# TimoLassmann/tagdust

Hardware: AMD Instinct MI355X
Metric: reads/s (150 bp, 8-barcode arch) (higher is better)
Workload: dtype f32

## Files before the change

tagdust_amd/csrc/td_api.hip:

```cpp
#include <math.h>
#include <stdarg.h>
#include <stdlib.h>
#include <string.h>
#include <unistd.h>

#include <mutex>
#include <thread>

#include "../../include/tagdust_model.h"
#include "td_ctx.h"
#include "td_model_flat.h"
#include "td_stats.h"

static std::string g_create_error;

static int g_hwq_user = 0;
static bool g_hwq_late = false;
static bool kfd_is_open()
{
	char path[64], target[64];
	for (int fd = 0; fd < 256; fd++) {
		snprintf(path, sizeof path, "/proc/self/fd/%d", fd);
		const ssize_t n = readlink(path, target, sizeof target - 1);
		if (n <= 0) continue;
// ... 10 lines not shown
}

int fail(td_ctx* c, const char* fmt, ...)
{
	char buf[512];
	va_list ap;
	va_start(ap, fmt);
	vsnprintf(buf, sizeof buf, fmt, ap);
	va_end(ap);
	if (c) c->err = buf; else g_create_error = buf;
	return TD_FAIL;
}

extern "C" const char* td_last_error(const td_ctx* ctx)
{
	return ctx ? ctx->err.c_str() : g_create_error.c_str();
}

extern "C" void td_stream_release(void);
static std::mutex g_live_mu;
static int g_live_ctx = 0;

extern "C" int td_ctx_create(int device, td_ctx** out)
{
	if (!out) return fail(nullptr, "td_ctx_create: out is NULL");
	*out = nullptr;
	int ndev = 0;
	hipError_t e = hipGetDeviceCount(&ndev);
	if (e != hipSuccess || ndev <= 0)
		return fail(nullptr, "td_ctx_create: no HIP device available (%s) -- this library has no CPU path",
		            e == hipSuccess ? "device count 0" : hipGetErrorString(e));
	if (device < 0 || device >= ndev) return fail(nullptr, "td_ctx_create: device %d out of range (0..%d)", device, ndev - 1);
	td_ctx* c = new td_ctx();
	c->device = device;
	hipDeviceProp_t prop;
	if (hipSetDevice(device) != hipSuccess || hipGetDeviceProperties(&prop, device) != hipSuccess) {
		delete c;
		return fail(nullptr, "td_ctx_create: cannot select device %d", device);
	}
	if (strncmp(prop.gcnArchName, "gfx950", 6) != 0) {
		std::string arch = prop.gcnArchName;
		delete c;
		return fail(nullptr, "td_ctx_create: device %d is %s; this library is built for gfx950 (MI355X) only", device, arch.c_str());
	}
	c->n_cu = prop.multiProcessorCount;
	if (const char* e = getenv("TD_SPECIALIZE")) c->spec.specialize = atoi(e) != 0;
	if (const char* e = getenv("TD_OVERLAP")) c->overlap = atoi(e) != 0;
	if (const char* e = getenv("TD_COMPACT_EGRESS")) c->compact_egress = atoi(e) != 0;
	if (const char* e = getenv("TD_RLE_CAP")) { const int v = atoi(e); if (v >= 1 && v <= 127) c->rle_cap_forced = v; }
	if (getenv("TD_NO_LENGTH_CLASSES")) c->length_classes = 0;
	if (getenv("TD_DEBUG_WAIT")) c->debug_wait = 1;
	if (getenv("TD_DEBUG_ALLOC")) c->debug_alloc = 1;
	if (const char* e = getenv("TD_WAVE_SLOTS")) { const long v = atol(e); if (v > 0) c->wave_slots_forced = v; }
	if (const char* e = getenv("TD_WS_CANDIDATES")) c->ws_candidates = atoi(e);
	if (const char* e = getenv("TD_SPEC_LSUM_LIMIT")) c->spec.lsum_limit = atof(e);
	if (getenv("TD_SPEC_SELFCHECK_FAIL")) c->spec.selfcheck_fail = 1;
	if (const char* e = getenv("TD_ASYNC_COMPILE")) c->spec.async_compile = atoi(e) != 0;
	c->hbm_total = prop.totalGlobalMem;
	bool ok = hipStreamCreateWithFlags(&c->stream, hipStreamNonBlocking) == hipSuccess &&
	          hipMalloc((void**)&c->d_logsum, sizeof(float) * TD_LOGSUM_LIVE) == hipSuccess &&
	          hipMalloc((void**)&c->d_counters, sizeof(unsigned long long) * TD_COUNTER_WORDS) == hipSuccess &&
	          hipMemcpy(c->d_logsum, td_logsum_table(), sizeof(float) * TD_LOGSUM_LIVE, hipMemcpyHostToDevice) == hipSuccess &&
	          hipMemset(c->d_counters, 0, sizeof(unsigned long long) * TD_COUNTER_WORDS) == hipSuccess;
	if (!ok) {
		td_ctx_destroy(c);
		return fail(nullptr, "td_ctx_create: HIP resource allocation failed: %s", hipGetErrorString(hipGetLastError()));
	}
	{ std::lock_guard<std::mutex> lk(g_live_mu); g_live_ctx++; c->counted = true; }
	*out = c;
	return TD_OK;
}

void free_dev_model(DevModel& d)
{
	void* p[] = { d.d_hdr, d.d_cols, d.d_hinfo, d.d_pred_off, d.d_pred_idx };
	for (void* q : p) if (q) (void)hipFree(q);
	d = DevModel();
}

extern "C" void td_ctx_destroy(td_ctx* c)
{
	if (!c) return;
	spec_retire_jobs(c, true);
	(void)hipSetDevice(c->device);
	hipStream_t streams[] = { c->stream, c->stream2, c->s_aux, c->s_fin, c->s_up, c->s_down };
	for (hipStream_t st : streams) if (st) (void)hipStreamSynchronize(st);
	free_dev_model(c->dev);
	census_release(c);
	mol_release(c);
	samples_release(c);
	void* bufs[] = { c->d_logsum, c->d_counters, c->d_ws, c->d_art_text, c->d_art_index, c->d_art_pk, c->d_art_seq, c->d_art_hits,
	                 c->spec.d_prune, c->d_tile_next, c->d_ws2, c->d_tile_next2 };
	for (void* p : bufs) if (p) (void)hipFree(p);
	for (int k = 0; k < TD_MAX_PIPELINE; k++) slot_release(c->slots[k]);
	if (c->ev_origin) (void)hipEventDestroy(c->ev_origin);
	(void)spec_unload(c);
	for (hipStream_t st : streams) if (st) (void)hipStreamDestroy(st);
	bool last = false;
	if (c->counted) { std::lock_guard<std::mutex> lk(g_live_mu); last = --g_live_ctx == 0; }
	delete c;
	if (last) td_stream_release();
}

int build_dev_model(td_ctx* c, const td_model_desc* m, DevModel& out)
{
	TdFlatModel f;
	std::string why;
	if (!td_flatten_model(m, f, why)) return fail(c, "%s", why.c_str());
	DevModel d;
	d.h = f.h;
	bool ok = hipMalloc((void**)&d.d_hdr, sizeof f.h) == hipSuccess && hipMalloc((void**)&d.d_cols, sizeof(TdCol) * f.cols.size()) == hipSuccess &&
	          hipMalloc((void**)&d.d_hinfo, sizeof(uint32_t) * f.hinfo.size()) == hipSuccess &&
	          hipMalloc((void**)&d.d_pred_off, sizeof(int32_t) * f.pred_off.size()) == hipSuccess &&
	          hipMalloc((void**)&d.d_pred_idx, sizeof(int32_t) * f.pred_idx.size()) == hipSuccess &&
	          hipMemcpy(d.d_hdr, &f.h, sizeof f.h, hipMemcpyHostToDevice) == hipSuccess &&
	          hipMemcpy(d.d_cols, f.cols.data(), sizeof(TdCol) * f.cols.size(), hipMemcpyHostToDevice) == hipSuccess &&
	          hipMemcpy(d.d_hinfo, f.hinfo.data(), sizeof(uint32_t) * f.hinfo.size(), hipMemcpyHostToDevice) == hipSuccess &&
	          hipMemcpy(d.d_pred_off, f.pred_off.data(), sizeof(int32_t) * f.pred_off.size(), hipMemcpyHostToDevice) == hipSuccess &&
	          hipMemcpy(d.d_pred_idx, f.pred_idx.data(), sizeof(int32_t) * f.pred_idx.size(), hipMemcpyHostToDevice) == hipSuccess;
	if (!ok) { free_dev_model(d); return fail(c, "td_model_upload: device tables: %s", hipGetErrorString(hipGetLastError())); }
	out = d;
	return TD_OK;
}

extern "C" int td_model_upload(td_ctx* c, const td_model_desc* m)
{
	if (!c || !m) return fail(c, "td_model_upload: NULL argument");
	HIPCHK(c, hipSetDevice(c->device));
	if (tickets_outstanding(c)) return fail(c, "td_model_upload: td_submit tickets are outstanding (td_wait them first)");
	spec_retire_jobs(c, false);
	DevModel dm;
	if (build_dev_model(c, m, dm) != TD_OK) return TD_FAIL;
	c->have_model = false;
	for (int k = 0; k < TD_MAX_PIPELINE; k++) { c->slots[k].staged = false; c->slots[k].ran = false; }
	HIPCHK(c, sync_compute(c));
	census_release(c);
	mol_release(c);
	samples_release(c);
	free_dev_model(c->dev);
	c->dev = dm;
	c->model.assign(m);
	c->half_slots = false;
	if (spec_model_uploaded(c) != TD_OK) return TD_FAIL;
	c->have_model = true;
	return TD_OK;
}

extern "C" int td_set_option(td_ctx* c, const char* name, int32_t value)
{
	if (!c || !name) return TD_FAIL;
	if (!strcmp(name, "specialize")) {
		c->spec.specialize = value != 0;
		return TD_OK;
	}
	if (!strcmp(name, "poison_workspace")) { c->poison = value != 0; return TD_OK; }
	if (!strcmp(name, "async_compile")) { c->spec.async_compile = value != 0; return TD_OK; }
	if (!strcmp(name, "spec_probe")) { c->spec.probe = value != 0; return TD_OK; }
	if (!strcmp(name, "compact_egress")) { c->compact_egress = value != 0; return TD_OK; }
	if (!strcmp(name, "stable_input")) {
		if (tickets_outstanding(c)) return fail(c, "td_set_option: stable_input cannot change while tickets are outstanding");
		c->stable_input = value != 0;
		return TD_OK;
	}
	if (!strcmp(name, "length_classes_enabled")) { c->length_classes = value != 0; return TD_OK; }
	if (!strcmp(name, "debug_wait")) { c->debug_wait = value != 0; return TD_OK; }
	if (!strcmp(name, "spec_lsum_limit")) { c->spec.lsum_limit = value > 0 ? (double)value : 1.0e6; return TD_OK; }
	if (!strcmp(name, "rle_cap")) {
		if (value < 0 || value > 127) return fail(c, "td_set_option: rle_cap must be 0 (default) .. 127");
		c->rle_cap_forced = value;
		return TD_OK;
	}
	if (!strcmp(name, "host_threads")) {
		if (value < 1 || value > 16) return fail(c, "td_set_option: host_threads must be 1..16");
		c->host_threads = value;
		return TD_OK;
	}
	if (!strcmp(name, "overlap_decode")) {
		if (tickets_outstanding(c)) return fail(c, "td_set_option: overlap_decode cannot change while tickets are outstanding");
		c->overlap = value != 0; c->submit_parity = 0;
		return TD_OK;
	}
	if (!strcmp(name, "pipeline_depth")) {
		if (value < 1 || value > TD_MAX_PIPELINE) return fail(c, "td_set_option: pipeline_depth must be 1..%d", TD_MAX_PIPELINE);
		if (tickets_outstanding(c)) return fail(c, "td_set_option: pipeline_depth cannot change while tickets are outstanding");
		c->pipeline_depth = value; c->next_slot = 0;
		return TD_OK;
	}
	return fail(c, "td_set_option: unknown option %s", name);
}

extern "C" int td_get_option(td_ctx* c, const char* name, int32_t* value)
{
	if (!c || !name || !value) return TD_FAIL;
	if (!strcmp(name, "specialize")) { *value = c->spec.specialize; return TD_OK; }
	if (!strcmp(name, "spec_lsum_clamped")) { *value = c->spec.ready && !c->spec.oob; return TD_OK; }
	if (!strcmp(name, "pipeline_depth")) { *value = c->pipeline_depth; return TD_OK; }
	if (!strcmp(name, "async_compile")) { *value = c->spec.async_compile; return TD_OK; }
	if (!strcmp(name, "spec_probe")) { *value = c->spec.probe; return TD_OK; }
	if (!strcmp(name, "spec_state")) { *value = spec_state_now(c); return TD_OK; }
	if (!strcmp(name, "spec_batches_generic")) { *value = c->spec.batches_generic; return TD_OK; }
	if (!strcmp(name, "spec_compiles_started")) { *value = td_spec_compiles_started(); return TD_OK; }
	if (!strcmp(name, "spec_probe_us")) { *value = c->spec.probe_us; return TD_OK; }
	if (!strcmp(name, "host_threads")) { *value = c->host_threads; return TD_OK; }
	if (!strcmp(name, "artifacts_active")) { *value = c->art_n > 0; return TD_OK; }
	if (!strcmp(name, "dust")) { *value = c->dust; return TD_OK; }
	if (!strcmp(name, "length_classes")) { *value = c->slots[c->last_slot].n_big; return TD_OK; }
	if (!strcmp(name, "overlap_decode")) { *value = c->overlap; return TD_OK; }
	if (!strcmp(name, "compact_egress")) { *value = c->compact_egress; return TD_OK; }
	if (!strcmp(name, "stable_input")) { *value = c->stable_input; return TD_OK; }
	if (!strcmp(name, "length_classes_enabled")) { *value = c->length_classes; return TD_OK; }
	if (!strcmp(name, "hw_queues")) { *value = g_hwq_user ? g_hwq_user : (g_hwq_late ? 4 : 8); return TD_OK; }
	if (!strcmp(name, "hw_queues_late")) { *value = g_hwq_late ? 1 : 0; return TD_OK; }
	if (!strcmp(name, "prune_active")) {
		*value = c->spec.ready && c->spec.prune_live && (c->spec.plan.prune_segs > 0 || c->spec.plan.sfx_first < c->spec.plan.S);
		return TD_OK;
	}
	if (!strcmp(name, "census_active")) { *value = c->census.on; return TD_OK; }
	if (!strcmp(name, "census_kernel_us")) return census_last_kernel_us(c, value);
	if (!strcmp(name, "samples")) { *value = c->samples.on ? c->samples.plan.n_samples : 0; return TD_OK; }
	if (!strcmp(name, "samples_kernel_us")) return samples_last_kernel_us(c, value);
	if (!strcmp(name, "molecules_active")) { *value = c->molecules.on; return TD_OK; }
	if (!strcmp(name, "dedup_active")) { *value = c->molecules.dedup.on; return TD_OK; }
	if (!strcmp(name, "dedup_frozen")) { *value = c->molecules.frozen.on; return TD_OK; }
	if (!strcmp(name, "mate_bases")) { *value = c->molecules.mate.bases; return TD_OK; }
	if (!strcmp(name, "mate_filter")) { *value = c->molecules.mate.filter ? 1 : 0; return TD_OK; }
	if (!strcmp(name, "collapse_active")) { *value = c->molecules.collapse.on; return TD_OK; }
	if (const int rc = mol_kernel_us(c, name, value); rc >= 0) return rc;
	if (!strcmp(name, "overlap_active")) {
		*value = c->overlap && c->pipeline_depth > 1 && c->spec.ready && c->stream2 != nullptr && c->d_ws2 != nullptr;
		return TD_OK;
	}
	return fail(c, "td_get_option: unknown option %s", name);
}

extern "C" int td_set_artifacts(td_ctx* c, const uint8_t* string, const int32_t* s_index, int32_t n_seq,
                                int32_t filter_error, int32_t n_threads)
{
	if (!c) return TD_FAIL;
	HIPCHK(c, hipSetDevice(c->device));
	if (c->d_art_text) { HIPCHK(c, hipFree(c->d_art_text)); c->d_art_text = nullptr; }
	if (c->d_art_index) { HIPCHK(c, hipFree(c->d_art_index)); c->d_art_index = nullptr; }
	if (c->d_art_pk) { HIPCHK(c, hipFree(c->d_art_pk)); c->d_art_pk = nullptr; }
	if (c->d_art_seq) { HIPCHK(c, hipFree(c->d_art_seq)); c->d_art_seq = nullptr; }
	if (c->d_art_hits) { HIPCHK(c, sync_compute(c)); HIPCHK(c, hipFree(c->d_art_hits)); c->d_art_hits = nullptr; }
	c->art_n = 0;
	if (n_seq <= 0) return TD_OK;
	if (!string || !s_index) return fail(c, "td_set_artifacts: null argument");
	if (n_threads < 1) return fail(c, "td_set_artifacts: n_threads = %d", n_threads);
	std::vector<int32_t> seq;
	std::vector<uint32_t> pk;
	std::string why;
	if (!td_pack_artifacts(string, s_index, n_seq, seq, pk, why)) return fail(c, "%s", why.c_str());
	const size_t bytes = (size_t)s_index[n_seq];
	HIPCHK(c, hipMalloc((void**)&c->d_art_text, bytes ? bytes : 1));
	HIPCHK(c, hipMalloc((void**)&c->d_art_index, sizeof(int32_t) * ((size_t)n_seq + 1)));
	if (bytes) HIPCHK(c, hipMemcpy(c->d_art_text, string, bytes, hipMemcpyHostToDevice));
	HIPCHK(c, hipMemcpy(c->d_art_index, s_index, sizeof(int32_t) * ((size_t)n_seq + 1), hipMemcpyHostToDevice));
	HIPCHK(c, hipMalloc((void**)&c->d_art_pk, pk.size() * 4));
	HIPCHK(c, hipMalloc((void**)&c->d_art_seq, seq.size() * 4));
	HIPCHK(c, hipMemcpy(c->d_art_pk, pk.data(), pk.size() * 4, hipMemcpyHostToDevice));
// ... 123 lines not shown
```

tagdust_amd/csrc/td_batch.hip:

```cpp
#include <stdlib.h>
#include <string.h>
#include <time.h>

#include "td_ctx.h"
#include "td_rnadust.h"

bool is_pinned(const void* p)
{
	if (!p) return false;
	hipPointerAttribute_t a;
	if (hipPointerGetAttributes(&a, p) != hipSuccess) { (void)hipGetLastError(); return false; }
	return a.type == hipMemoryTypeHost;
}

static void parallel_copy(td_ctx* c, void* dst, const void* src, size_t bytes)
{
	c->pool.copy(dst, src, bytes, c->host_threads);
}

static int slot_events(td_ctx* c, TdSlot& s)
{
	if (s.ev_k0) return TD_OK;
	HIPCHK(c, hipEventCreate(&s.ev_k0));
	HIPCHK(c, hipEventCreate(&s.ev_k1));
	HIPCHK(c, hipEventCreateWithFlags(&s.ev_up, hipEventDisableTiming));
	HIPCHK(c, hipEventCreateWithFlags(&s.ev_done, hipEventDisableTiming));
	HIPCHK(c, hipEventCreateWithFlags(&s.ev_down, hipEventDisableTiming));
	HIPCHK(c, hipEventCreateWithFlags(&s.ev_pack, hipEventDisableTiming));
	HIPCHK(c, hipEventCreateWithFlags(&s.ev_hits, hipEventDisableTiming));
	return TD_OK;
}

void slot_release(TdSlot& s)
{
	void* dev[] = { s.d_raw, s.d_offs, s.d_read_at, s.d_keys, s.d_vals, s.d_sort_tmp, s.d_packed, s.d_lens, s.d_art_left,
	                s.d_out, s.d_res, s.d_seq, s.d_lab, s.d_keepo, s.d_rle, s.d_runs, s.d_judged, s.d_mate_raw, s.d_mate_offs, s.d_mate_w,
	                s.d_mate_n, s.d_mate_type };
	for (void* p : dev) if (p) (void)hipFree(p);
	void* pinned[] = { s.h_raw, s.h_offs, s.h_res, s.h_seq, s.h_lab, s.h_keepo, s.h_rle, s.h_mate_raw, s.h_mate_offs };
	for (void* p : pinned) if (p) (void)hipHostFree(p);
	hipEvent_t ev[] = { s.ev_up, s.ev_k0, s.ev_k1, s.ev_done, s.ev_down, s.ev_pack, s.ev_hits };
	for (hipEvent_t e : ev) if (e) (void)hipEventDestroy(e);
	s = TdSlot();
}

static int hbm_free(td_ctx* c, size_t& free_b)
{
	size_t total_b = 0;
	HIPCHK(c, hipMemGetInfo(&free_b, &total_b));
	return TD_OK;
}

static int ensure_workspace(td_ctx* c, TdSlot& s)
{
	if (spec_before_batch(c, s.lmax) != TD_OK) return TD_FAIL;
	make_layout(s.lay, c->dev.h.S, c->dev.h.H, c->dev.h.C, s.lmax, c->dev.h.max_ncol);
	TdWsRequest rq;
	rq.small_slot_bytes = rq.big_slot_bytes = s.lay.slot_bytes;
	if (c->spec.ready) {
		td_spec_layout(s.slay, c->spec.plan, s.n_long > 0 ? s.lmax_small : s.lmax);
		td_spec_layout(s.slay_big, c->spec.plan, s.lmax);
		rq.small_slot_bytes = s.slay.slot_bytes; rq.big_slot_bytes = s.slay_big.slot_bytes;
	}
	rq.n_tiles = s.n_tiles; rq.n_long = s.n_long; rq.lmax_small = s.lmax_small; rq.lmax = s.lmax;
	rq.wpb = (c->spec.ready ? c->spec.block : td_kernel_block_threads()) / TD_WAVE;
	rq.want_slots = c->wave_slots_forced > 0 ? c->wave_slots_forced : (int64_t)c->n_cu * (c->spec.ready ? c->spec.waves_per_cu : 2 * rq.wpb);
	rq.spec_ready = c->spec.ready; rq.pipelined = s.pipelined; rq.overlap = c->overlap; rq.pipeline_depth = c->pipeline_depth;
	rq.half_slots = c->half_slots; rq.wsi = s.wsi;
	rq.cap_ws = c->cap_ws; rq.cap_ws2 = c->cap_ws2; rq.ws_candidates = c->ws_candidates;
	const TdWsPlan p = plan_workspace(rq, [](void* ctx, size_t* free_b) { return hbm_free((td_ctx*)ctx, *free_b) == TD_OK; }, c);
	c->half_slots = p.half_slots;
	if (p.overlap_given_up) { c->overlap = 0; s.wsi = 0; s.cs = c->stream; }
	s.n_long = p.n_long; s.lmax_small = p.lmax_small; s.n_big = p.n_big;
	if (p.one_geometry) s.slay = s.slay_big;
	if (p.query_failed) return TD_FAIL;
	if (p.no_fit) return fail(c, "td_batch_upload: workspace of %lld bytes per wave does not fit in HBM", (long long)p.ws_slot_bytes);
	if (p.alloc_bytes > 0) {
		uint8_t*& ws = s.wsi ? c->d_ws2 : c->d_ws;
		size_t& cap_ws = s.wsi ? c->cap_ws2 : c->cap_ws;
		const size_t need = p.alloc_bytes;
		HIPCHK(c, sync_compute(c));
		if (p.n_candidates <= 1) {
			if (ensure(c, &ws, &cap_ws, need) != TD_OK) return TD_FAIL;
		} else {
			if (ws) { HIPCHK(c, hipFree(ws)); ws = nullptr; cap_ws = 0; }
			uint8_t* cand[4] = { nullptr, nullptr, nullptr, nullptr };
			float ms[4] = { 0, 0, 0, 0 };
			int n_ok = 0, best = -1;
			for (int k = 0; k < p.n_candidates; k++) {
				if (hipMalloc((void**)&cand[k], need) != hipSuccess) { (void)hipGetLastError(); cand[k] = nullptr; break; }
				n_ok++;
			}
			for (int k = 0; k < n_ok; k++) {
				if (td_ws_probe(cand[k], p.ws_slot_bytes, p.n_wave_slots, c->stream, &ms[k]) != hipSuccess) ms[k] = 1e30f;
				if (best < 0 || ms[k] < ms[best]) best = k;
			}
			if (best < 0) return fail(c, "td_batch_upload: workspace of %zu bytes could not be allocated", need);
			if (c->debug_alloc) fprintf(stderr, "tagdust_hip: workspace candidates: probe %.2f %.2f %.2f %.2f ms -> #%d\n", ms[0], ms[1], ms[2], ms[3], best);
			for (int k = 0; k < n_ok; k++) if (k != best) (void)hipFree(cand[k]);
			ws = cand[best]; cap_ws = need;
		}
	}
	s.n_wave_slots = p.n_wave_slots;
	s.ws_slot_bytes = p.ws_slot_bytes;
	s.ws_bytes = p.ws_bytes;
	return TD_OK;
}

static int slot_stage(td_ctx* c, TdSlot& s, const TdRoute& route, const void* bases, int is_ascii, const int64_t* offs, int64_t n, hipStream_t up, bool with_workspace = true, bool take_mate = false)
{
	s.reset_staged(route);
	if (with_workspace && !c->have_model) return fail(c, "td_batch_upload: no model uploaded");
	if (!offs || n < 0 || (!bases && n > 0 && offs[n] > offs[0])) return fail(c, "td_batch_upload: bad arguments");
	if (n > 0x7fffffffLL - TD_WAVE) return fail(c, "td_batch_upload: %lld reads in one batch", (long long)n);
	HIPCHK(c, hipSetDevice(c->device));
	if (slot_events(c, s) != TD_OK) return TD_FAIL;
	const int64_t base = offs[0];
	if (ensure_pinned(c, &s.h_offs, &s.cap_h_offs, (size_t)(n + 1) * 8) != TD_OK) return TD_FAIL;
	int lmax = 1, lmin = 0x7fffffff;
	int64_t bad = -1;
	s.h_offs[0] = 0;
	for (int64_t i = 0; i < n; i++) {
		const int64_t l = offs[i + 1] - offs[i];
		s.h_offs[i + 1] = offs[i + 1] - base;
		if (l < 0 || l > 100000) { bad = i; break; }
		if (l > lmax) lmax = (int)l;
		if (l < lmin) lmin = (int)l;
	}
	if (bad >= 0) return fail(c, "td_batch_upload: read %lld has length %lld", (long long)bad, (long long)(offs[bad + 1] - offs[bad]));
	const int64_t n_bases = n > 0 ? offs[n] - base : 0;
	const int64_t n_tiles = (n + TD_WAVE - 1) / TD_WAVE;
	const TdLengthClasses lc = plan_length_classes(offs, n, lmin, lmax, n_tiles, c->spec.ready && with_workspace && c->length_classes);
	s.n_long = lc.n_long; s.lmax_small = lc.lmax_small;
	const int nw2 = (lmax + 15) / 16, nw1 = (lmax + 31) / 32;
	const bool sorted = n > 0 && lmin != lmax;

	const size_t n_packed = (size_t)(n_tiles * (int64_t)(nw2 + nw1) * TD_WAVE), n_lanes = (size_t)(n_tiles * TD_WAVE);
	const OutLayout ol = out_layout(n_tiles, lmax, nw1);
	if (ensure(c, &s.d_raw, &s.cap_raw, (size_t)n_bases) != TD_OK || ensure(c, &s.d_offs, &s.cap_offs, (size_t)(n + 1) * 8) != TD_OK ||
	    ensure(c, &s.d_packed, &s.cap_packed, n_packed * 4) != TD_OK || ensure(c, &s.d_lens, &s.cap_lens, n_lanes * 4) != TD_OK ||
	    ensure(c, &s.d_art_left, &s.cap_art_left, n_lanes) != TD_OK || ensure(c, &s.d_out, &s.cap_out, (size_t)ol.total) != TD_OK)
		return TD_FAIL;
	size_t sort_tmp = 0;
	if (sorted) {
		sort_tmp = td_stage_sort_temp_bytes(n, lmax);
		if (ensure(c, &s.d_read_at, &s.cap_read_at, (size_t)n * 4) != TD_OK || ensure(c, &s.d_keys, &s.cap_keys, (size_t)n * 8) != TD_OK ||
		    ensure(c, &s.d_vals, &s.cap_vals, (size_t)n * 4) != TD_OK || ensure(c, &s.d_sort_tmp, &s.cap_sort_tmp, sort_tmp) != TD_OK)
			return TD_FAIL;
	}
	s.lmax = lmax; s.nw2 = nw2; s.nw1 = nw1; s.n_tiles = (int32_t)n_tiles;
	if (with_workspace && ensure_workspace(c, s) != TD_OK) { s.n_tiles = 0; return TD_FAIL; }
	s.for_spec = with_workspace && c->spec.ready;
	s.n_tiles = 0;

	const void* src = (const uint8_t*)bases + base;
	s.raw_direct = n_bases > 0 && is_pinned(src);
// ... 357 lines not shown

extern "C" int td_batch_download(td_ctx* c, td_read_result* res, int8_t* labels, uint8_t* seq_out)
{
	if (!c) return TD_FAIL;
	TdSlot& s = c->slots[0];
	HIPCHK(c, hipSetDevice(c->device));
	if (slot_fetch_begin(c, s, res, labels, seq_out, false) != TD_OK) return TD_FAIL;
	return slot_fetch_end(c, s);
}

extern "C" int td_submit(td_ctx* c, const void* bases, int32_t is_ascii, const int64_t* offs, int64_t n_reads, int mode,
                         td_read_result* res, int8_t* labels, uint8_t* seq_out, int64_t* ticket)
{
	if (!c || !ticket) return fail(c, "td_submit: NULL argument");
	*ticket = 0;
	HIPCHK(c, hipSetDevice(c->device));
	if (!c->s_up) {
		int lo = 0, hi = 0;
		HIPCHK(c, hipDeviceGetStreamPriorityRange(&lo, &hi));
		HIPCHK(c, hipStreamCreateWithFlags(&c->s_up, hipStreamNonBlocking));
		HIPCHK(c, hipStreamCreateWithPriority(&c->s_down, hipStreamNonBlocking, hi));
		HIPCHK(c, hipStreamCreateWithPriority(&c->s_aux, hipStreamNonBlocking, hi));
		HIPCHK(c, hipStreamCreateWithPriority(&c->s_fin, hipStreamNonBlocking, hi));
	}
	int k = -1;
	for (int j = 0; j < c->pipeline_depth; j++) {
		const int cand = (c->next_slot + j) % c->pipeline_depth;
		if (!c->slots[cand].ticket) { k = cand; break; }
	}
	if (k < 0) return fail(c, "td_submit: all %d pipeline slots hold batches that have not been waited for", c->pipeline_depth);
	if (mode == TD_MODE_RNA_DUST && labels) return fail(c, "td_submit: TD_MODE_RNA_DUST has no labels (pass NULL)");
	if (spec_handover(c, false) != TD_OK) return TD_FAIL;
	const bool take_mate = c->molecules.mate.bases > 0 && mode == TD_MODE_GET_LABEL;
	if (take_mate && mol_mate_check(c, n_reads, "td_submit") != TD_OK) return TD_FAIL;
	TdSlot& s = c->slots[k];
	TdRoute rt = sync_route(c);
	rt.pipelined = true;
	if (c->overlap && c->pipeline_depth > 1 && c->spec.ready) {
		if (!c->stream2) HIPCHK(c, hipStreamCreateWithFlags(&c->stream2, hipStreamNonBlocking));
		if (c->submit_parity) { rt.cs = c->stream2; rt.wsi = 1; }
		c->submit_parity ^= 1;
		rt.aux = c->s_aux; rt.fin = c->s_fin;
	}
	if (slot_stage(c, s, rt, bases, is_ascii != 0, offs, n_reads, c->s_up, mode != TD_MODE_RNA_DUST, take_mate) != TD_OK) return TD_FAIL;
	if (slot_decode(c, s, mode, labels != nullptr) != TD_OK) return TD_FAIL;
	if (slot_fetch_begin(c, s, res, labels, seq_out, true) != TD_OK) return TD_FAIL;
	if ((s.raw_direct || s.mate_direct) && !c->stable_input) HIPCHK(c, hipEventSynchronize(s.ev_up));
	s.ticket = ++c->ticket_counter;
	c->next_slot = (k + 1) % c->pipeline_depth;
	*ticket = s.ticket;
	return TD_OK;
}

extern "C" int td_wait(td_ctx* c, int64_t ticket)
{
	if (!c) return TD_FAIL;
	HIPCHK(c, hipSetDevice(c->device));
	for (int k = 0; k < TD_MAX_PIPELINE; k++) {
		TdSlot& s = c->slots[k];
		if (ticket != 0 && s.ticket == ticket) {
			const int rc = slot_fetch_end(c, s);
			s.ticket = 0;
			c->last_slot = k;
			return rc;
		}
	}
	return fail(c, "td_wait: no batch with ticket %lld is in flight", (long long)ticket);
}

extern "C" int td_arch_scores(td_ctx* c, const td_model_desc* const* models, int32_t n_models, const uint8_t* codes,
                              const int64_t* offs, int64_t n_reads, float* b_scores)
{
	if (!c || !models || n_models < 1 || !offs || !b_scores || n_reads < 0) return fail(c, "td_arch_scores: bad arguments");
	if (tickets_outstanding(c)) return fail(c, "td_arch_scores: td_submit tickets are outstanding (td_wait them first)");
	HIPCHK(c, hipSetDevice(c->device));
	TdSlot& s = c->slots[0];
	const TdRoute rt = sync_route(c);
	if (slot_stage(c, s, rt, codes, 0, offs, n_reads, c->stream, false) != TD_OK) return TD_FAIL;
	s.staged = false;
	if (s.n_tiles == 0) return TD_OK;
	const int wpb = td_kernel_block_threads() / TD_WAVE;
	const int64_t n_lanes = (int64_t)s.n_tiles * TD_WAVE;
	const int64_t wave_budget = (int64_t)c->n_cu * 2 * wpb;
	std::vector<DevModel> dm((size_t)n_models);
	int rc = TD_OK;
	float* d_b = nullptr;
	TdKernelArgs* d_args = nullptr;
	std::vector<float> h_b;
	std::vector<int32_t> h_read_at;
	auto cleanup = [&]() {
		for (auto& d : dm) free_dev_model(d);
		if (d_b) (void)hipFree(d_b);
		if (d_args) (void)hipFree(d_args);
	};
	if (hipMalloc((void**)&d_b, sizeof(float) * (size_t)(n_lanes * n_models)) != hipSuccess ||
	    hipMalloc((void**)&d_args, sizeof(TdKernelArgs) * (size_t)n_models) != hipSuccess) { cleanup(); return fail(c, "td_arch_scores: out of device memory"); }
	size_t free_b = 0, total_b = 0;
	if (hipMemGetInfo(&free_b, &total_b) != hipSuccess) { cleanup(); return fail(c, "td_arch_scores: hipMemGetInfo failed"); }
	const int64_t ws_budget = (int64_t)((double)(free_b + c->cap_ws) * 0.85);
	std::vector<TdKernelArgs> args((size_t)n_models);
	int k0 = 0;
	while (k0 < n_models && rc == TD_OK) {
		int k1 = k0;
		int64_t ws_total = 0;
		std::vector<int64_t> ws_off;
		int max_slots = 0;
		int chunk = n_models - k0;
		for (;;) {
			int64_t per = wave_budget / chunk / wpb * wpb;
			if (per < wpb) per = wpb;
			int64_t cap = ((int64_t)s.n_tiles + wpb - 1) / wpb * wpb;
			if (per > cap) per = cap;
			ws_total = 0; ws_off.clear(); max_slots = (int)per;
// ... 93 lines not shown
```

tagdust_amd/csrc/td_batch_plan.cpp:

```cpp
#include "td_batch_plan.h"

#include "../../include/tagdust_hip.h"

#include <vector>

int64_t align256(int64_t v) { return (v + 255) & ~(int64_t)255; }

void make_layout(TdWsLayout& L, int S, int H, int C, int lmax, int max_ncol)
{
	int64_t o = 0;
	L.codes = o; o = align256(o + (int64_t)(lmax + 2) * TD_WAVE);
	L.sb = o;    o = align256(o + (int64_t)(S + 1) * (lmax + 2) * TD_WAVE * 4);
	L.sf = o;    o = align256(o + (int64_t)(S + 1) * (lmax + 2) * TD_WAVE * 4);
	L.bw = o;    o = align256(o + (int64_t)C * lmax * TD_WAVE * 8);
	L.fwrow = o; o = align256(o + (int64_t)max_ncol * TD_WAVE * 8);
	L.dp = o;    o = align256(o + (int64_t)lmax * H * TD_WAVE * 4);
	L.path = o;  o = align256(o + (int64_t)lmax * H * TD_WAVE);
	L.acc = o;   o = align256(o + (int64_t)H * TD_WAVE * 4);
	L.total = o; o = align256(o + (int64_t)H * TD_WAVE * 4);
	L.dust = o;  o = align256(o + (int64_t)64 * TD_WAVE);
	L.slot_bytes = o;
}

OutLayout out_layout(int64_t n_tiles, int lmax, int nw1)
{
	OutLayout o;
	o.soa_stride = n_tiles * TD_WAVE * 4;
	int64_t p = 8 * o.soa_stride;
	o.keep = p; p = align256(p + n_tiles * nw1 * TD_WAVE * 4);
	o.labels = p; p = align256(p + n_tiles * (int64_t)(lmax + 1) * TD_WAVE);
	o.total = p;
	return o;
}

TdLengthClasses plan_length_classes(const int64_t* offs, int64_t n, int lmin, int lmax, int64_t n_tiles, bool wanted)
{
	TdLengthClasses lc = { 0, lmax };
	if (!wanted || lmin == lmax || n_tiles < 64) return lc;
	std::vector<int64_t> hist((size_t)lmax + 2, 0);
	for (int64_t i = 0; i < n; i++) hist[(size_t)(offs[i + 1] - offs[i])]++;
	const int64_t t99 = n_tiles - 1 - (n_tiles + 99) / 100;
	const int64_t rank = t99 * TD_WAVE + TD_WAVE - 1;
	int64_t acc = 0;
	int l99 = lmax;
	for (int l = 0; l <= lmax; l++) { acc += hist[(size_t)l]; if (acc > rank) { l99 = l; break; } }
	if (l99 < 1) l99 = 1;
	if ((int64_t)lmax * 2 >= (int64_t)l99 * 3) {
		int64_t upto = 0;
		for (int l = 0; l <= l99; l++) upto += hist[(size_t)l];
		const int64_t first_long_tile = upto / TD_WAVE;
		lc.n_long = (int32_t)(n_tiles - first_long_tile);
		lc.lmax_small = l99;
	}
	return lc;
}

TdWsPlan plan_workspace(const TdWsRequest& rq, TdFreeMemFn free_mem, void* arg)
{
	TdWsPlan p;
	p.half_slots = rq.half_slots;
	int overlap = rq.overlap, wsi = rq.wsi;
	for (;;) {
		p.n_long = rq.n_long; p.lmax_small = rq.lmax_small;
		p.one_geometry = false;
		int64_t slot_bytes = rq.small_slot_bytes;
		const int wpb = rq.wpb;
		int64_t slots = rq.want_slots;
		if (slots > rq.n_tiles) slots = rq.n_tiles;
		if (slots < 1) slots = 1;
		slots = (slots + wpb - 1) / wpb * wpb;
		p.n_big = 0;
		int64_t big_extra = 0;
		if (rq.spec_ready && p.n_long > 0) {
			if ((int64_t)p.n_long * 4 <= slots) {
				p.n_big = p.n_long;
				big_extra = (int64_t)p.n_big * (rq.big_slot_bytes - rq.small_slot_bytes);
			} else {
				p.n_long = 0; p.lmax_small = rq.lmax;
				p.one_geometry = true;
				slot_bytes = rq.big_slot_bytes;
			}
		}
		p.ws_slot_bytes = slot_bytes;
		const size_t cap_ws = wsi ? rq.cap_ws2 : rq.cap_ws;
		if (rq.pipelined && overlap && rq.pipeline_depth > 1 && rq.spec_ready && !p.half_slots) {
			size_t free_b = 0;
			if (!free_mem(arg, &free_b)) { p.query_failed = true; return p; }
			const double avail = (double)free_b + (double)rq.cap_ws + (double)rq.cap_ws2;
			if (2.0 * (double)(slots * slot_bytes + big_extra) > 0.8 * avail && (double)(slots * slot_bytes + big_extra) <= 0.8 * avail) p.half_slots = true;
		}
		if (p.half_slots && rq.pipelined) {
			int64_t half = (slots / 2 + wpb - 1) / wpb * wpb;
			if (half < wpb) half = wpb;
			if (half >= p.n_big * 4 || p.n_big == 0) slots = half;
		}
		if ((size_t)(slots * slot_bytes + big_extra) > cap_ws) {
			size_t free_b = 0;
			if (!free_mem(arg, &free_b)) { p.query_failed = true; return p; }
			if (wsi == 1 && (double)(slots * slot_bytes + big_extra) > (p.half_slots ? 0.6 : 0.4) * (double)(free_b + cap_ws)) {
				p.overlap_given_up = true;
				overlap = 0; wsi = 0;
				continue;
			}
			const int64_t budget = (int64_t)((double)(free_b + cap_ws) * 0.85);
			if (slots * slot_bytes + big_extra > budget) {
				if (big_extra > budget / 2) {
					p.n_long = 0; p.lmax_small = rq.lmax; p.n_big = 0; big_extra = 0;
					p.one_geometry = true;
					slot_bytes = rq.big_slot_bytes;
					p.ws_slot_bytes = slot_bytes;
				}
				slots = (budget - big_extra) / slot_bytes / wpb * wpb;
			}
			if (slots < wpb || slots < p.n_big) { p.no_fit = true; return p; }
			if ((size_t)(slots * slot_bytes + big_extra) > cap_ws) {
				p.alloc_bytes = (size_t)(slots * slot_bytes + big_extra);
				p.n_candidates = rq.ws_candidates;
				if (p.n_candidates > 4) p.n_candidates = 4;
				if (p.alloc_bytes < ((size_t)2 << 30) || (double)p.alloc_bytes * p.n_candidates > 0.6 * (double)(free_b + cap_ws)) p.n_candidates = 1;
			}
		}
		p.n_wave_slots = (int32_t)slots;
		p.ws_bytes = slots * slot_bytes + big_extra;
		return p;
	}
}

static TdEgressChannel plain_channel(int k, size_t bytes, TdPageLockedFn page_locked, void* arg)
{
	TdEgressChannel ch;
	ch.form = page_locked(arg, k) ? TD_EG_DIRECT : TD_EG_STAGED;
	ch.copy_bytes = ch.alloc_bytes = bytes;
	return ch;
}

static TdEgressChannel compact_channel(size_t copy_bytes, size_t alloc_bytes)
{
	TdEgressChannel ch;
	ch.form = TD_EG_COMPACT;
	ch.copy_bytes = copy_bytes; ch.alloc_bytes = alloc_bytes;
	return ch;
}

TdEgressPlan plan_egress(const TdEgressRequest& rq, TdPageLockedFn page_locked, void* arg)
{
	TdEgressPlan p;
	if (rq.n_reads == 0) return p;
// ... 26 lines not shown
```

tagdust_amd/csrc/td_batch_plan.h:

```cpp
#pragma once
#include <stddef.h>
#include <stdint.h>

#include "td_device.h"

#ifndef TD_HIDDEN
#define TD_HIDDEN __attribute__((visibility("hidden")))
#endif

TD_HIDDEN int64_t align256(int64_t v);
TD_HIDDEN void make_layout(TdWsLayout& L, int S, int H, int C, int lmax, int max_ncol);
struct OutLayout { int64_t soa_stride, keep, labels, total; };
TD_HIDDEN OutLayout out_layout(int64_t n_tiles, int lmax, int nw1);

struct TdLengthClasses { int32_t n_long, lmax_small; };
TD_HIDDEN TdLengthClasses plan_length_classes(const int64_t* offs, int64_t n, int lmin, int lmax, int64_t n_tiles, bool wanted);

struct TdWsRequest {
	int64_t n_tiles = 0;
	int32_t n_long = 0, lmax_small = 0, lmax = 0;
	int64_t small_slot_bytes = 0, big_slot_bytes = 0;
	int wpb = 1;
	int64_t want_slots = 0;
	bool spec_ready = false, pipelined = false;
	int overlap = 0, pipeline_depth = 1;
	bool half_slots = false;
	int wsi = 0;
	size_t cap_ws = 0, cap_ws2 = 0;
	int ws_candidates = 1;
};
struct TdWsPlan {
	int32_t n_wave_slots = 0, n_big = 0, n_long = 0, lmax_small = 0;
	bool one_geometry = false;
	int64_t ws_slot_bytes = 0, ws_bytes = 0;
	bool half_slots = false;
	bool overlap_given_up = false;
	size_t alloc_bytes = 0;
	int n_candidates = 1;
	bool no_fit = false;
	bool query_failed = false;
};
typedef bool (*TdFreeMemFn)(void* arg, size_t* free_bytes);
TD_HIDDEN TdWsPlan plan_workspace(const TdWsRequest& rq, TdFreeMemFn free_mem, void* arg);

enum { TD_CH_RES = 0, TD_CH_SEQ = 1, TD_CH_LAB = 2, TD_N_CHANNELS = 3 };
enum { TD_EG_NONE = 0, TD_EG_COMPACT, TD_EG_DIRECT, TD_EG_STAGED };
struct TdEgressRequest {
	int64_t n_reads = 0, n_bases = 0;
	int32_t nw1 = 0, n_tiles = 0;
	bool want[TD_N_CHANNELS] = { false, false, false };
	bool compact_egress = false;
	bool raw_host = false;
	int32_t runs_cap = 0;
	int32_t rle_capacity = 0;
};
struct TdEgressChannel {
	int form = TD_EG_NONE;
	size_t copy_bytes = 0;
	size_t alloc_bytes = 0;
};
struct TdEgressPlan {
	TdEgressChannel ch[TD_N_CHANNELS];
	int32_t rle_cap = 0;
	size_t rle_flag_word = 0;
	bool finish_reads_runs = false;
	size_t runs_flag_word = 0;
	size_t lab_plain_bytes = 0;
};
typedef bool (*TdPageLockedFn)(void* arg, int channel);
TD_HIDDEN TdEgressPlan plan_egress(const TdEgressRequest& rq, TdPageLockedFn page_locked, void* arg);
TD_HIDDEN void plan_labels_plain(TdEgressPlan& p, TdPageLockedFn page_locked, void* arg);
```

tagdust_amd/csrc/td_ctx.h:

```cpp
#pragma once
#include <hip/hip_runtime.h>
#include <stdio.h>
#include <memory>
#include <string>
#include <vector>
#include "../../include/tagdust_hip.h"
#include "td_device.h"
#include "td_batch_plan.h"
#include "td_jit.h"
#include "td_stage.h"
#include "td_host_inner.h"
#include "td_census.h"
#include "td_molecules.h"
#include "td_samples.h"

#define TD_HIDDEN __attribute__((visibility("hidden")))
#define TD_MAX_PIPELINE 4
#define TD_COUNTER_WORDS (TD_NUM_COUNTERS + TD_NUM_DIAG_COUNTERS)

struct TdRoute {
	hipStream_t cs = nullptr;
	hipStream_t aux = nullptr;
	hipStream_t fin = nullptr;
	int wsi = 0;
	bool pipelined = false;
};
struct TdStaged : TdRoute {
	int64_t n_reads = 0, n_bases = 0;
	int32_t n_tiles = 0, lmax = 0, nw2 = 0, nw1 = 0;
	int is_ascii = 0;
	bool sorted = false;
	bool staged = false;
	bool for_spec = false;
	bool raw_direct = false;
	int32_t mate_m = 0;
	bool mate_direct = false;
	bool mate_judged = false;
	bool mate_typed = false;
	int32_t samples_gen = 0;
	const uint8_t* raw_host = nullptr;
	TdStageBatch sb{};
	TdWsLayout lay{};
	TdSpecLayout slay{};
	int32_t n_wave_slots = 0;
	int64_t ws_slot_bytes = 0;
	int32_t n_long = 0, lmax_small = 0, n_big = 0;
	TdSpecLayout slay_big{};
	int64_t ws_bytes = 0;
};
struct TdDecoded {
	int mode = 0;
	bool ran = false;
	float last_ms = -1.0f;
	int32_t runs_cap = 0;
	bool hits_queued = false;
};
struct TdFetch {
	td_read_result* u_res = nullptr; int8_t* u_labels = nullptr; uint8_t* u_seq = nullptr;
	TdEgressPlan plan;
	bool copies_deferred = false;
	bool finished = false;
};
struct TdSlot : TdStaged, TdDecoded, TdFetch {
	int64_t ticket = 0;
	void reset_staged(const TdRoute& r) { static_cast<TdStaged&>(*this) = TdStaged(); static_cast<TdRoute&>(*this) = r; reset_decoded(); }
	void reset_decoded() { static_cast<TdDecoded&>(*this) = TdDecoded(); reset_fetch(); }
	void reset_fetch() { static_cast<TdFetch&>(*this) = TdFetch(); }
	uint8_t* d_raw = nullptr;      size_t cap_raw = 0;
	int64_t* d_offs = nullptr;     size_t cap_offs = 0;
	int32_t* d_read_at = nullptr;  size_t cap_read_at = 0;
	uint32_t* d_keys = nullptr;    size_t cap_keys = 0;
	int32_t* d_vals = nullptr;     size_t cap_vals = 0;
	uint8_t* d_sort_tmp = nullptr; size_t cap_sort_tmp = 0;
	uint32_t* d_packed = nullptr;  size_t cap_packed = 0;
	int32_t* d_lens = nullptr;     size_t cap_lens = 0;
	uint8_t* d_art_left = nullptr; size_t cap_art_left = 0;
	uint8_t* d_out = nullptr;      size_t cap_out = 0;
	uint8_t* d_res = nullptr;      size_t cap_res = 0;
	uint8_t* d_seq = nullptr;      size_t cap_seq = 0;
	int8_t*  d_lab = nullptr;      size_t cap_lab = 0;
	uint32_t* d_keepo = nullptr;   size_t cap_keepo = 0;
	uint32_t* d_rle = nullptr;     size_t cap_rle = 0;
	uint32_t* d_runs = nullptr;    size_t cap_runs = 0;
	int32_t* d_judged = nullptr;   size_t cap_judged = 0;
	uint8_t* d_mate_raw = nullptr; size_t cap_mate_raw = 0;
	int64_t* d_mate_offs = nullptr; size_t cap_mate_offs = 0;
	unsigned long long* d_mate_w = nullptr; size_t cap_mate_w = 0;
	uint8_t* d_mate_n = nullptr;   size_t cap_mate_n = 0;
	int32_t* d_mate_type = nullptr; size_t cap_mate_type = 0;
	uint8_t* h_mate_raw = nullptr; size_t cap_h_mate_raw = 0;
	int64_t* h_mate_offs = nullptr; size_t cap_h_mate_offs = 0;
	uint32_t* h_keepo = nullptr;   size_t cap_h_keepo = 0;
	uint32_t* h_rle = nullptr;     size_t cap_h_rle = 0;
	uint8_t* h_raw = nullptr;      size_t cap_h_raw = 0;
	int64_t* h_offs = nullptr;     size_t cap_h_offs = 0;
	uint8_t* h_res = nullptr;      size_t cap_h_res = 0;
	uint8_t* h_seq = nullptr;      size_t cap_h_seq = 0;
// ... 49 lines not shown
	int selfcheck_fail = 0;
	float* d_prune = nullptr;   int prune_lcap = 0, prune_stride = 0;
	bool prune_live = false;
};

struct td_ctx {
	int device = 0;
	int host_threads = td_context_threads();
	TdWorkers pool;
	hipStream_t stream = nullptr;
	std::string err;
	int n_cu = 0;
	size_t hbm_total = 0;

	bool have_model = false;
	ModelCopy model;
	DevModel dev;
	float* d_logsum = nullptr;
	unsigned long long* d_counters = nullptr;
	TdSpecState spec;

	float threshold = 0.0f;
	int32_t minlen = 16, dust = 100;

	uint8_t* d_art_text = nullptr; int32_t* d_art_index = nullptr;
	uint32_t* d_art_pk = nullptr; int32_t* d_art_seq = nullptr;
	int32_t art_n = 0, art_fe = 0, art_threads = 1;
	unsigned long long* d_art_hits = nullptr;
	TdCensusState census;
	TdMolState molecules;
	TdSamplesState samples;
	int64_t win_first = 0, win_total = 0;
	int32_t match_start = 0, match_len = 0;
	TdSlot slots[TD_MAX_PIPELINE];
	int pipeline_depth = 3, next_slot = 0, last_slot = 0;
	bool counted = false;
	int poison = 0;
	int compact_egress = 1;
	int stable_input = 0;
	int rle_cap_forced = 0;
	int length_classes = 1;
	int debug_wait = 0;
	int debug_alloc = 0;
	long wave_slots_forced = 0;
	int ws_candidates = 3;
	int64_t ticket_counter = 0;
	hipStream_t s_up = nullptr, s_down = nullptr;
	uint8_t* d_ws = nullptr;      size_t cap_ws = 0;
	hipStream_t stream2 = nullptr;
	hipStream_t s_aux = nullptr, s_fin = nullptr;
	uint8_t* d_ws2 = nullptr;     size_t cap_ws2 = 0;
	int overlap = 1, submit_parity = 0;
	bool half_slots = false;
	int32_t* d_tile_next = nullptr, * d_tile_next2 = nullptr;
	hipEvent_t ev_origin = nullptr;
};

TD_HIDDEN int fail(td_ctx* c, const char* fmt, ...);
TD_HIDDEN bool is_pinned(const void* p);
TD_HIDDEN bool tickets_outstanding(const td_ctx* c);
TD_HIDDEN void slot_release(TdSlot& s);
TD_HIDDEN int build_dev_model(td_ctx* c, const td_model_desc* m, DevModel& out);
TD_HIDDEN void free_dev_model(DevModel& d);

#define HIPCHK(c, call)                                                                       \
	do {                                                                                      \
		hipError_t e_ = (call);                                                               \
		if (e_ != hipSuccess) return fail((c), "%s failed: %s", #call, hipGetErrorString(e_)); \
	} while (0)

static hipError_t sync_compute(td_ctx* c)
{
	hipError_t e = hipStreamSynchronize(c->stream);
	if (e == hipSuccess && c->stream2) e = hipStreamSynchronize(c->stream2);
	if (e == hipSuccess && c->s_aux) e = hipStreamSynchronize(c->s_aux);
	if (e == hipSuccess && c->s_fin) e = hipStreamSynchronize(c->s_fin);
	return e;
}

static int wait_compute(td_ctx* c)
{
	HIPCHK(c, hipSetDevice(c->device));
	HIPCHK(c, sync_compute(c));
	return TD_OK;
}

template <typename T>
static int ensure(td_ctx* c, T** p, size_t* cap, size_t bytes)
{
	if (*cap >= bytes && *p) return TD_OK;
	if (*p) { HIPCHK(c, hipFree(*p)); *p = nullptr; *cap = 0; }
	if (bytes == 0) bytes = 256;
	HIPCHK(c, hipMalloc((void**)p, bytes));
	*cap = bytes;
	if (c && c->debug_alloc && bytes > (1u << 30)) fprintf(stderr, "tagdust_hip: hipMalloc(%zu) = %p\n", bytes, (void*)*p);
	return TD_OK;
}

template <typename T>
static int ensure_pinned(td_ctx* c, T** p, size_t* cap, size_t bytes)
{
	if (*cap >= bytes && *p) return TD_OK;
	if (*p) { HIPCHK(c, hipHostFree(*p)); *p = nullptr; *cap = 0; }
	if (bytes == 0) bytes = 256;
	bytes += bytes / 4;
	HIPCHK(c, hipHostMalloc((void**)p, bytes, hipHostMallocPortable));
// ... 47 lines not shown
```

Before: 82.89 million.

## Halve wave slots for side-by-side overlapping launches when pipeline is device-bound

Adds a side_by_side mode that, under pipelined overlap with specialized kernels and depth >= 3, shrinks each batch's wave-slot count to half. Two concurrent streams can then share the GPU's CUs instead of each trying to fill it. In the default adaptive mode (2), td_wait times how long the host blocks on the device event. After three consecutive device-dominated waits it marks the context device-bound and enables the halved geometry. This adds an extra event synchronize on the wait path and risks lower per-batch occupancy if the two launches do not actually overlap.

```diff
diff --git a/tagdust_amd/csrc/td_api.hip b/tagdust_amd/csrc/td_api.hip
--- a/tagdust_amd/csrc/td_api.hip
+++ b/tagdust_amd/csrc/td_api.hip
@@ -86,6 +86,7 @@
 	if (getenv("TD_DEBUG_WAIT")) c->debug_wait = 1;
 	if (getenv("TD_DEBUG_ALLOC")) c->debug_alloc = 1;
 	if (const char* e = getenv("TD_WAVE_SLOTS")) { const long v = atol(e); if (v > 0) c->wave_slots_forced = v; }
+	if (const char* e = getenv("TD_SIDE_BY_SIDE")) { const int v = atoi(e); if (v >= 0 && v <= 2) c->side_by_side = v; }
 	if (const char* e = getenv("TD_WS_CANDIDATES")) c->ws_candidates = atoi(e);
 	if (const char* e = getenv("TD_SPEC_LSUM_LIMIT")) c->spec.lsum_limit = atof(e);
 	if (getenv("TD_SPEC_SELFCHECK_FAIL")) c->spec.selfcheck_fail = 1;
@@ -175,6 +176,7 @@
 	c->dev = dm;
 	c->model.assign(m);
 	c->half_slots = false;
+	c->pace_reset();
 	if (spec_model_uploaded(c) != TD_OK) return TD_FAIL;
 	c->have_model = true;
 	return TD_OK;
@@ -212,12 +214,20 @@
 	if (!strcmp(name, "overlap_decode")) {
 		if (tickets_outstanding(c)) return fail(c, "td_set_option: overlap_decode cannot change while tickets are outstanding");
 		c->overlap = value != 0; c->submit_parity = 0;
+		c->pace_reset();
+		return TD_OK;
+	}
+	if (!strcmp(name, "side_by_side")) {
+		if (value < 0 || value > 2) return fail(c, "td_set_option: side_by_side must be 0, 1 or 2");
+		c->side_by_side = value;
+		c->pace_reset();
 		return TD_OK;
 	}
 	if (!strcmp(name, "pipeline_depth")) {
 		if (value < 1 || value > TD_MAX_PIPELINE) return fail(c, "td_set_option: pipeline_depth must be 1..%d", TD_MAX_PIPELINE);
 		if (tickets_outstanding(c)) return fail(c, "td_set_option: pipeline_depth cannot change while tickets are outstanding");
 		c->pipeline_depth = value; c->next_slot = 0;
+		c->pace_reset();
 		return TD_OK;
 	}
 	return fail(c, "td_set_option: unknown option %s", name);
@@ -240,6 +250,8 @@
 	if (!strcmp(name, "dust")) { *value = c->dust; return TD_OK; }
 	if (!strcmp(name, "length_classes")) { *value = c->slots[c->last_slot].n_big; return TD_OK; }
 	if (!strcmp(name, "overlap_decode")) { *value = c->overlap; return TD_OK; }
+	if (!strcmp(name, "side_by_side")) { *value = c->side_by_side; return TD_OK; }
+	if (!strcmp(name, "side_by_side_active")) { *value = c->slots[c->last_slot].side_by_side; return TD_OK; }
 	if (!strcmp(name, "compact_egress")) { *value = c->compact_egress; return TD_OK; }
 	if (!strcmp(name, "stable_input")) { *value = c->stable_input; return TD_OK; }
 	if (!strcmp(name, "length_classes_enabled")) { *value = c->length_classes; return TD_OK; }
diff --git a/tagdust_amd/csrc/td_batch.hip b/tagdust_amd/csrc/td_batch.hip
--- a/tagdust_amd/csrc/td_batch.hip
+++ b/tagdust_amd/csrc/td_batch.hip
@@ -68,6 +68,7 @@
 	rq.spec_ready = c->spec.ready; rq.pipelined = s.pipelined; rq.overlap = c->overlap; rq.pipeline_depth = c->pipeline_depth;
 	rq.half_slots = c->half_slots; rq.wsi = s.wsi;
 	rq.cap_ws = c->cap_ws; rq.cap_ws2 = c->cap_ws2; rq.ws_candidates = c->ws_candidates;
+	rq.side_by_side = c->side_by_side == 1 || (c->side_by_side == 2 && c->device_bound);
 	const TdWsPlan p = plan_workspace(rq, [](void* ctx, size_t* free_b) { return hbm_free((td_ctx*)ctx, *free_b) == TD_OK; }, c);
 	c->half_slots = p.half_slots;
 	if (p.overlap_given_up) { c->overlap = 0; s.wsi = 0; s.cs = c->stream; }
@@ -102,6 +103,7 @@
 		}
 	}
 	s.n_wave_slots = p.n_wave_slots;
+	s.side_by_side = p.side_by_side;
 	s.ws_slot_bytes = p.ws_slot_bytes;
 	s.ws_bytes = p.ws_bytes;
 	return TD_OK;
@@ -565,6 +567,19 @@
 	return TD_OK;
 }
 
+static int note_device_wait(td_ctx* c, TdSlot& s)
+{
+	const double t0 = wall_ms();
+	HIPCHK(c, hipEventSynchronize(s.ev_done));
+	const double t1 = wall_ms();
+	const bool waited = c->last_done_ms > 0.0 && (t1 - t0) * 4.0 >= t1 - c->last_done_ms;
+	c->waited_run = waited ? c->waited_run + 1 : 0;
+	if (c->debug_wait) fprintf(stderr, "td_wait: %.2f of %.2f ms for the device, %d in a row\n", t1 - t0, c->last_done_ms > 0.0 ? t1 - c->last_done_ms : 0.0, c->waited_run);
+	c->last_done_ms = t1;
+	if (c->waited_run >= 3) c->device_bound = true;
+	return TD_OK;
+}
+
 extern "C" int td_wait(td_ctx* c, int64_t ticket)
 {
 	if (!c) return TD_FAIL;
@@ -572,6 +587,8 @@
 	for (int k = 0; k < TD_MAX_PIPELINE; k++) {
 		TdSlot& s = c->slots[k];
 		if (ticket != 0 && s.ticket == ticket) {
+			const bool full_overlapping_launch = s.ran && s.for_spec && s.n_tiles > 0 && c->overlap && c->stream2 && !c->half_slots && !s.side_by_side;
+			if (c->side_by_side == 2 && !c->device_bound && full_overlapping_launch && s.finished && s.copies_deferred && note_device_wait(c, s) != TD_OK) return TD_FAIL;
 			const int rc = slot_fetch_end(c, s);
 			s.ticket = 0;
 			c->last_slot = k;
diff --git a/tagdust_amd/csrc/td_batch_plan.cpp b/tagdust_amd/csrc/td_batch_plan.cpp
--- a/tagdust_amd/csrc/td_batch_plan.cpp
+++ b/tagdust_amd/csrc/td_batch_plan.cpp
@@ -62,7 +62,7 @@
 	int overlap = rq.overlap, wsi = rq.wsi;
 	for (;;) {
 		p.n_long = rq.n_long; p.lmax_small = rq.lmax_small;
-		p.one_geometry = false;
+		p.one_geometry = false; p.side_by_side = false;
 		int64_t slot_bytes = rq.small_slot_bytes;
 		const int wpb = rq.wpb;
 		int64_t slots = rq.want_slots;
@@ -93,6 +93,12 @@
 			int64_t half = (slots / 2 + wpb - 1) / wpb * wpb;
 			if (half < wpb) half = wpb;
 			if (half >= p.n_big * 4 || p.n_big == 0) slots = half;
+		} else if (rq.side_by_side && rq.pipelined && overlap && rq.spec_ready && rq.pipeline_depth >= 3) {
+			int64_t full = rq.want_slots < 1 ? 1 : rq.want_slots;
+			full = (full + wpb - 1) / wpb * wpb;
+			int64_t half = (full / 2 + wpb - 1) / wpb * wpb;
+			if (half < wpb) half = wpb;
+			if (rq.n_tiles > full / 2 && half < slots && (half >= p.n_big * 4 || p.n_big == 0)) { slots = half; p.side_by_side = true; }
 		}
 		if ((size_t)(slots * slot_bytes + big_extra) > cap_ws) {
 			size_t free_b = 0;
diff --git a/tagdust_amd/csrc/td_batch_plan.h b/tagdust_amd/csrc/td_batch_plan.h
--- a/tagdust_amd/csrc/td_batch_plan.h
+++ b/tagdust_amd/csrc/td_batch_plan.h
@@ -28,12 +28,14 @@
 	int wsi = 0;
 	size_t cap_ws = 0, cap_ws2 = 0;
 	int ws_candidates = 1;
+	bool side_by_side = false;
 };
 struct TdWsPlan {
 	int32_t n_wave_slots = 0, n_big = 0, n_long = 0, lmax_small = 0;
 	bool one_geometry = false;
 	int64_t ws_slot_bytes = 0, ws_bytes = 0;
 	bool half_slots = false;
+	bool side_by_side = false;
 	bool overlap_given_up = false;
 	size_t alloc_bytes = 0;
 	int n_candidates = 1;
diff --git a/tagdust_amd/csrc/td_ctx.h b/tagdust_amd/csrc/td_ctx.h
--- a/tagdust_amd/csrc/td_ctx.h
+++ b/tagdust_amd/csrc/td_ctx.h
@@ -43,6 +43,7 @@
 	TdWsLayout lay{};
 	TdSpecLayout slay{};
 	int32_t n_wave_slots = 0;
+	bool side_by_side = false;
 	int64_t ws_slot_bytes = 0;
 	int32_t n_long = 0, lmax_small = 0, n_big = 0;
 	TdSpecLayout slay_big{};
@@ -198,6 +199,11 @@
 	uint8_t* d_ws2 = nullptr;     size_t cap_ws2 = 0;
 	int overlap = 1, submit_parity = 0;
 	bool half_slots = false;
+	int side_by_side = 2;
+	bool device_bound = false;
+	int waited_run = 0;
+	double last_done_ms = 0.0;
+	void pace_reset() { device_bound = false; waited_run = 0; last_done_ms = 0.0; }
 	int32_t* d_tile_next = nullptr, * d_tile_next2 = nullptr;
 	hipEvent_t ev_origin = nullptr;
 };
```

Result: faster. 85.95 million (median of 6 runs) (+3.7%).
